# lesliegaga/GPT-SoVITS

Measured on AMD Instinct MI355X. Metric: synthesised audio sec/sec (1/RTF), v2 pipeline, higher is better.
Workload: dtype f16

## Files before the change

gpt-sovits_amd/csrc/conv_wide.hip:

```cpp
#include <stdio.h>
#include <stdlib.h>

#include <algorithm>
#include <type_traits>

#include "common.h"

namespace gsv {

namespace {

typedef _Float16 T;
typedef h8 F;
typedef _Float16 T4 __attribute__((ext_vector_type(4)));

__device__ __forceinline__ void mma32w(f16v& acc, const h8& a, const h8& b) { acc = __builtin_amdgcn_mfma_f32_32x32x16_f16(a, b, acc, 0, 0, 0); }
__device__ __forceinline__ h8 lrelu8w(h8 v, float s) { h8 t = v * (_Float16)s; return __builtin_elementwise_max(v, t); }
__device__ __forceinline__ h8 relu8w(h8 v) { return __builtin_elementwise_max(v, (h8){0, 0, 0, 0, 0, 0, 0, 0}); }

template <bool RES, bool ACCU, int NW>
__global__ __launch_bounds__(NW * 64) void conv_wide_f16_kernel(ConvArgs a, int rows_win, int ntiles) {
  constexpr int G = 8, KC = 16, CC = 128, CT = 128, TM = 2, TN = NW == 8 ? 2 : 4, WN = NW == 8 ? 4 : 2, NT = NW * 64;
  constexpr int LDX = CC + G, VPR = CC / G;
  constexpr int WLOADS = CT * VPR / NT;
  constexpr int XB = (306 * VPR + NT - 1) / NT;
  constexpr int LDO = CT + 4, PR = TN * 32, IPR = CT / 4, NI = PR * IPR / NT;
  extern __shared__ __attribute__((aligned(16))) unsigned char smem[];
  T* xs = (T*)smem;
  T* ws = xs + (size_t)306 * LDX;
  float* os = (float*)smem;
  static_assert((size_t)PR * LDO * 4 <= (size_t)306 * LDX * 2, "epilogue tile must fit in the window");
  const int tid = threadIdx.x, lane = tid & 63, wave = tid >> 6;
  const int r = lane & 31, h = lane >> 5;
  const int wm = wave / WN, wn = wave % WN;
  const T* __restrict__ x = (const T*)a.x;
  const T* __restrict__ w = (const T*)a.w;
  const int total = rows_win * VPR;
  const int ecg = tid % IPR, ec = 4 * ecg;
  f4 ebias = (f4){0.f, 0.f, 0.f, 0.f};
  if (a.bias) for (int j = 0; j < 4; ++j) ebias[j] = a.bias[ec + j];

  auto load_w = [&](int tap, F* regs) {
#pragma unroll
    for (int i = 0; i < WLOADS; ++i) {
      const int v = tid + i * NT;
      const int row = v / VPR, col = v - row * VPR;
      regs[i] = *(const F*)(w + (long long)row * a.ldw + (long long)tap * CC + col * G);
    }
  };
  auto store_w = [&](int buf, const F* regs) {
#pragma unroll
    for (int i = 0; i < WLOADS; ++i) {
      const int v = tid + i * NT;
      const int row = v / VPR, col = v - row * VPR;
      *(F*)(ws + ((size_t)buf * CT + row) * LDX + col * G) = regs[i];
    }
  };
  auto load_window = [&](int tile, F* regs) {
    const int win_start = tile * 256 - a.pad;
#pragma unroll
    for (int i = 0; i < XB; ++i) {
      const int v = min(tid + i * NT, total - 1);
      const int row = v / VPR, col = v - row * VPR;
      const int ti = win_start + row;
      const F val = *(const F*)(x + (long long)min(max(ti, 0), a.T_in - 1) * a.ldx + col * G);
      regs[i] = (ti >= 0 && ti < a.T_in) ? val : (F){0, 0, 0, 0, 0, 0, 0, 0};
    }
  };
  auto store_window = [&](const F* regs) {
#pragma unroll
    for (int i = 0; i < XB; ++i) {
      const int v = tid + i * NT;
      if (v < total) {
        const int row = v / VPR, col = v - row * VPR;
        F val = regs[i];
        if (a.pre_act == ACT_LRELU) val = lrelu8w(val, a.pre_slope);
        else if (a.pre_act == ACT_RELU) val = relu8w(val);
        *(F*)(xs + (size_t)row * LDX + col * G) = val;
      }
    }
  };
  int tile = blockIdx.x;
  {
    F first[XB], w0[WLOADS];
    load_window(min(tile, ntiles - 1), first);
    load_w(0, w0);
    store_window(first);
    store_w(0, w0);
  }
  lds_barrier();
  for (; tile < ntiles; tile += gridDim.x) {
    const int t0 = tile * 256;
    const bool pf = a.prof && blockIdx.x == 100 && tile == 100 + 3 * (int)gridDim.x && tid == 0;
    int pi = 0;
#define WSTAMP() do { if (pf) a.prof[pi++] = __builtin_amdgcn_s_memrealtime(); } while (0)
    WSTAMP();
    F nxt[XB];
    load_window(min(tile + (int)gridDim.x, ntiles - 1), nxt);
    T4 rv[RES ? NI : 1];
    auto load_res_pass = [&](int pass) {
#pragma unroll
      for (int e = 0; e < (RES ? NI : 0); ++e) {
        const int t = min(t0 + pass * PR + (tid + e * NT) / IPR, a.T_out - 1);
        rv[e] = *(const T4*)((const T*)a.res + (long long)t * a.ldr + ec);
      }
    };
    if (RES) load_res_pass(0);
    f16v acc[TM][TN];
#pragma unroll
    for (int m = 0; m < TM; ++m)
#pragma unroll
      for (int n = 0; n < TN; ++n)
#pragma unroll
        for (int i = 0; i < 16; ++i) acc[m][n][i] = 0.f;
    for (int tap = 0; tap < a.taps; ++tap) {
      const int buf = tap & 1;
      F wnx[WLOADS];
      const bool more = tap + 1 < a.taps;
      if (more) load_w(tap + 1, wnx);
      const int shift = tap * a.dil;
      const T* wb = ws + (size_t)buf * CT * LDX;
#pragma unroll 2
      for (int ks = 0; ks < CC / KC; ++ks) {
        const int kk = ks * KC + G * h;
        F af[TM], bf[TN];
#pragma unroll
        for (int m = 0; m < TM; ++m) af[m] = *(const F*)(wb + (size_t)((wm * TM + m) * 32 + r) * LDX + kk);
#pragma unroll
        for (int n = 0; n < TN; ++n) bf[n] = *(const F*)(xs + (size_t)((wn * TN + n) * 32 + r + shift) * LDX + kk);
#pragma unroll
        for (int m = 0; m < TM; ++m)
#pragma unroll
          for (int n = 0; n < TN; ++n) mma32w(acc[m][n], af[m], bf[n]);
      }
      if (more) {
        store_w(buf ^ 1, wnx);
        lds_barrier();
      }
      WSTAMP();
    }
#pragma unroll
    for (int pass = 0; pass < WN; ++pass) {
      lds_barrier();
      WSTAMP();
      if (wn == pass) {
#pragma unroll
        for (int m = 0; m < TM; ++m)
#pragma unroll
          for (int n = 0; n < TN; ++n) {
            const int tl = n * 32 + r;
#pragma unroll
            for (int g = 0; g < 4; ++g) {
              const int cl = (wm * TM + m) * 32 + 8 * g + 4 * h;
              *(f4*)(os + (size_t)tl * LDO + cl) = (f4){acc[m][n][4 * g], acc[m][n][4 * g + 1], acc[m][n][4 * g + 2], acc[m][n][4 * g + 3]};
            }
          }
      }
      WSTAMP();
      lds_barrier();
      WSTAMP();
      T4 ya[ACCU ? NI : 1];
#pragma unroll
      for (int e = 0; e < (ACCU ? NI : 0); ++e) {
        const int t = min(t0 + pass * PR + (tid + e * NT) / IPR, a.T_out - 1);
        ya[e] = *(const T4*)((const T*)a.y + (long long)t * a.ldy + ec);
      }
      auto items = [&](auto act_tag) {
#pragma unroll
        for (int e = 0; e < NI; ++e) {
          const int tl = (tid + e * NT) / IPR;
          const int t = t0 + pass * PR + tl;
          if (t >= a.T_out) continue;
          const f4 av = *(const f4*)(os + (size_t)tl * LDO + 4 * ecg);
          float v[4];
#pragma unroll
          for (int j = 0; j < 4; ++j) {
            float u = av[j] + ebias[j];
            if (RES) u += (float)rv[e][j];
            u *= a.scale;
            u = post_act_c<decltype(act_tag)::value>(a.post_act, u);
            if (ACCU) u += (float)ya[e][j];
            v[j] = u;
          }
          *(T4*)((T*)a.y + (long long)t * a.ldy + ec) = (T4){(T)v[0], (T)v[1], (T)v[2], (T)v[3]};
        }
      };
      GSV_ACT_DISPATCH(a.post_act, items);
      if (RES && pass + 1 < WN) load_res_pass(pass + 1);
      WSTAMP();
    }
    F w0[WLOADS];
    load_w(0, w0);
    lds_barrier();
    store_window(nxt);
    store_w(0, w0);
    lds_barrier();
    WSTAMP();
  }
}

}

int launch_conv_wide(int dtype, const ConvArgs& a, hipStream_t s) {
  static const bool off = getenv("GSV_NO_CONV_WIDE") != nullptr;
  if (off || dtype != GSV_F16) return 1;
  if (a.Cin != 128 || a.Cout != 128 || a.Z != 1 || a.stride != 1 || a.ups_u > 0 || a.dil < 1 || a.gate || a.taps < 2) return 1;
  if (a.out_f32 || a.res_f32 || a.y_col0 != 0 || a.T_virt < 16384 || a.T_out != a.T_virt || a.T_in < 1) return 1;
  if (a.ldx % 8 != 0 || a.ldw % 8 != 0 || a.ldy % 4 != 0 || (a.res && a.ldr % 4 != 0) || ((uintptr_t)a.x % 16) || ((uintptr_t)a.w % 16)) return 1;
  const int span = (a.taps - 1) * a.dil;
  if (span > 50 || a.pad < 0 || a.pad > span) return 1;
  const int rows_win = 256 + span;
  const int ntiles = cdiv(a.T_virt, 256);
  const size_t lds = ((size_t)306 + 2 * 128) * 136 * 2;
  const int grid = std::min(ntiles, 256);
  ConvArgs b = a;
  static unsigned long long* d_prof = nullptr;
  static int prof_calls = 0;
  if (getenv("GSV_WIDE_PROF") && !d_prof) { (void)hipMalloc((void**)&d_prof, 64 * 8); (void)hipMemset(d_prof, 0, 64 * 8); }
  b.prof = d_prof;
  const bool res = a.res != nullptr, acc = a.accumulate != 0;
  static const int nw = getenv("GSV_WIDE_WAVES") ? atoi(getenv("GSV_WIDE_WAVES")) : 8;
#define GSV_WIDE_NW(R, A, W)                                                                                               \
  do {                                                                                                                     \
    auto kern = conv_wide_f16_kernel<R, A, W>;                                                                             \
    static bool set = false;                                                                                               \
    if (!set) { GSV_HIP(hipFuncSetAttribute((const void*)kern, hipFuncAttributeMaxDynamicSharedMemorySize, 160 * 1024)); set = true; } \
    hipLaunchKernelGGL(kern, dim3(grid), dim3(W * 64), lds, s, b, rows_win, ntiles);                                       \
  } while (0)
#define GSV_WIDE(R, A) do { if (nw == 8) GSV_WIDE_NW(R, A, 8); else GSV_WIDE_NW(R, A, 4); } while (0)
  if (res && acc) GSV_WIDE(true, true);
  else if (res) GSV_WIDE(true, false);
  else if (acc) GSV_WIDE(false, true);
  else GSV_WIDE(false, false);
#undef GSV_WIDE
#undef GSV_WIDE_NW
  GSV_HIP(hipGetLastError());
  if (d_prof && ++prof_calls == 3) {
    (void)hipStreamSynchronize(s);
    unsigned long long hp[64];
    (void)hipMemcpy(hp, d_prof, sizeof(hp), hipMemcpyDeviceToHost);
    fprintf(stderr, "[wide prof] taps %d:", a.taps);
    for (int i = 1; i < 24 && hp[i]; ++i) fprintf(stderr, " %.2f", (double)(hp[i] - hp[0]) / 100.0);
    fprintf(stderr, "\n");
  }
  return GSV_OK;
}

}
```

Before: 2789.

## Add persistent ring-pipelined conv kernel for 128/256-channel dilated convolutions

Adds a new persistent conv kernel that double-buffers weight slabs per tap and spreads the next tile's input window loads across the taps. This overlaps global loads with MFMA work. It extends coverage to Cin/Cout of 256 by looping over input-channel chunks and splitting output halves across blocks, and it reuses a weight slab for the epilogue staging. It runs first by default for 3/7/11-tap convs, with the old wide kernel kept as a fallback. The risks are extra barriers per tap and higher register pressure from the per-tap template unrolling.

```diff
diff --git a/gpt-sovits_amd/csrc/conv_wide.hip b/gpt-sovits_amd/csrc/conv_wide.hip
--- a/gpt-sovits_amd/csrc/conv_wide.hip
+++ b/gpt-sovits_amd/csrc/conv_wide.hip
@@ -3,6 +3,7 @@
 
 #include <algorithm>
 #include <type_traits>
+#include <utility>
 
 #include "common.h"
 
@@ -197,13 +198,271 @@
     lds_barrier();
     WSTAMP();
   }
-}
-
+#undef WSTAMP
+}
+
+template <int... I, class Fn> __device__ __forceinline__ void static_for(std::integer_sequence<int, I...>, Fn&& f) {
+  (f(std::integral_constant<int, I>{}), ...);
+}
+
+template <bool RES, bool ACCU, int TAPS>
+__global__ __launch_bounds__(512) void conv_ring_f16_kernel(ConvArgs a, int rows_win, int ntiles, int nch, int nh) {
+  constexpr int NW = 8, G = 8, KC = 16, CC = 128, CT = 128, TM = 2, TN = 2, WN = 4, NT = NW * 64;
+  constexpr int LDX = CC + G, VPR = CC / G;
+  constexpr int WLOADS = CT * VPR / NT;
+  constexpr int XB = (306 * VPR + NT - 1) / NT;
+  constexpr int LDO = CT + 4, PR = TN * 32, IPR = CT / 4, NI = PR * IPR / NT;
+  extern __shared__ __attribute__((aligned(16))) unsigned char smem[];
+  T* xs = (T*)smem;
+  T* ws = xs + (size_t)306 * LDX;
+  static_assert((size_t)PR * LDO * 4 <= (size_t)CT * LDX * 2, "epilogue pass must fit in a weight slab");
+  const int tid = threadIdx.x, lane = tid & 63, wave = tid >> 6;
+  const int r = lane & 31, h = lane >> 5;
+  const int wm = wave / WN, wn = wave % WN;
+  const T* __restrict__ x = (const T*)a.x;
+  const T* __restrict__ w = (const T*)a.w;
+  const int total = rows_win * VPR;
+  const int half = nh == 2 ? (blockIdx.x >> 3) & 1 : 0;
+  const int cout0 = half * CT;
+  const int tstep = nh == 2 ? (int)gridDim.x / 2 : (int)gridDim.x;
+  int tile = nh == 2 ? (blockIdx.x >> 4) * 8 + (blockIdx.x & 7) : blockIdx.x;
+  if (tile >= ntiles) return;
+  const int ecg = tid % IPR, ec = cout0 + 4 * ecg;
+
+  auto opaque = [](int v) { asm volatile("" : "+s"(v)); return v; };
+  auto load_w = [&](int tap, int c, F* regs) {
+    const int ldw = opaque(a.ldw);
+#pragma unroll
+    for (int i = 0; i < WLOADS; ++i) {
+      const int v = tid + i * NT;
+      const int row = v / VPR, col = v - row * VPR;
+      regs[i] = *(const F*)(w + (long long)(cout0 + row) * ldw + (long long)tap * a.Cin + c * CC + col * G);
+    }
+  };
+  auto store_w = [&](int buf, const F* regs) {
+#pragma unroll
+    for (int i = 0; i < WLOADS; ++i) {
+      const int v = tid + i * NT;
+      const int row = v / VPR, col = v - row * VPR;
+      *(F*)(ws + ((size_t)buf * CT + row) * LDX + col * G) = regs[i];
+    }
+  };
+  auto load_window = [&](int tl, int c, F* regs, auto i0, auto i1) {
+    const int win_start = tl * 256 - a.pad;
+    const int ldx = opaque(a.ldx);
+#pragma unroll
+    for (int i = decltype(i0)::value; i < decltype(i1)::value; ++i) {
+      const int v = min(tid + i * NT, total - 1);
+      const int row = v / VPR, col = v - row * VPR;
+      const int ti = win_start + row;
+      regs[i] = *(const F*)(x + (long long)min(max(ti, 0), a.T_in - 1) * ldx + c * CC + col * G);
+    }
+  };
+  auto store_window = [&](int tl, const F* regs) {
+    const int win_start = tl * 256 - a.pad;
+#pragma unroll
+    for (int i = 0; i < XB; ++i) {
+      const int v = tid + i * NT;
+      if (v < total) {
+        const int row = v / VPR, col = v - row * VPR;
+        const int ti = win_start + row;
+        F val = (ti >= 0 && ti < a.T_in) ? regs[i] : (F){0, 0, 0, 0, 0, 0, 0, 0};
+        if (a.pre_act == ACT_LRELU) val = lrelu8w(val, a.pre_slope);
+        else if (a.pre_act == ACT_RELU) val = relu8w(val);
+        *(F*)(xs + (size_t)row * LDX + col * G) = val;
+      }
+    }
+  };
+  {
+    F first[XB], w0[WLOADS];
+    load_window(tile, 0, first, std::integral_constant<int, 0>{}, std::integral_constant<int, XB>{});
+    load_w(0, 0, w0);
+    store_window(tile, first);
+    store_w(0, w0);
+  }
+  lds_barrier();
+  int pbuf = 0;
+  for (int it = 0; tile < ntiles; tile += tstep, ++it) {
+    const int t0 = tile * 256;
+    const bool pf = a.prof && blockIdx.x == 100 && it == 1 && tid == 0;
+    int pi = 0;
+#define RSTAMP() do { if (pf) a.prof[pi++] = __builtin_amdgcn_s_memrealtime(); } while (0)
+    RSTAMP();
+    const int ntile = tile + tstep < ntiles ? tile + tstep : tile;
+    T4 rv[RES ? NI : 1], yv[ACCU ? NI : 1];
+    f4 ebias = (f4){0.f, 0.f, 0.f, 0.f};
+    auto load_epi_pass = [&](int pass) {
+#pragma unroll
+      for (int e = 0; e < NI; ++e) {
+        const int t = min(t0 + pass * PR + (tid + e * NT) / IPR, a.T_out - 1);
+        if (RES) rv[e] = *(const T4*)((const T*)a.res + (long long)t * a.ldr + ec);
+        if (ACCU && !RES) yv[e] = *(const T4*)((const T*)a.y + (long long)t * a.ldy + ec);
+      }
+    };
+    f16v acc[TM][TN];
+#pragma unroll
+    for (int m = 0; m < TM; ++m)
+#pragma unroll
+      for (int n = 0; n < TN; ++n)
+#pragma unroll
+        for (int i = 0; i < 16; ++i) acc[m][n][i] = 0.f;
+    int last_buf = 0;
+    for (int c = 0; c < nch; ++c) {
+      const bool last = c + 1 == nch;
+      const int nc = last ? 0 : c + 1, nt = last ? ntile : tile;
+      F nxt[XB];
+      static_for(std::make_integer_sequence<int, TAPS>{}, [&](auto tap_c) {
+        constexpr int tap = decltype(tap_c)::value;
+        const int buf = pbuf ^ (tap & 1);
+        F wnx[WLOADS];
+        if (tap + 1 < TAPS) load_w(tap + 1, c, wnx);
+        else load_w(0, nc, wnx);
+        load_window(nt, nc, nxt, std::integral_constant<int, tap * XB / TAPS>{}, std::integral_constant<int, (tap + 1) * XB / TAPS>{});
+        if (tap == TAPS - 2 && last) {
+          if (a.bias) ebias = *(const f4*)(a.bias + ec);
+          load_epi_pass(0);
+        }
+        const int shift = tap * opaque(a.dil);
+        const T* wb = ws + (size_t)buf * CT * LDX;
+#pragma unroll 2
+        for (int ks = 0; ks < CC / KC; ++ks) {
+          const int kk = ks * KC + G * h;
+          F af[TM], bf[TN];
+#pragma unroll
+          for (int m = 0; m < TM; ++m) af[m] = *(const F*)(wb + (size_t)((wm * TM + m) * 32 + r) * LDX + kk);
+#pragma unroll
+          for (int n = 0; n < TN; ++n) bf[n] = *(const F*)(xs + (size_t)((wn * TN + n) * 32 + r + shift) * LDX + kk);
+#pragma unroll
+          for (int m = 0; m < TM; ++m)
+#pragma unroll
+            for (int n = 0; n < TN; ++n) mma32w(acc[m][n], af[m], bf[n]);
+        }
+        if (tap + 1 < TAPS) {
+          store_w(buf ^ 1, wnx);
+          lds_barrier();
+        } else {
+          lds_barrier();
+          store_window(nt, nxt);
+          store_w(buf ^ 1, wnx);
+          last_buf = buf;
+          if (!last) lds_barrier();
+        }
+        RSTAMP();
+      });
+      pbuf = last_buf ^ 1;
+    }
+    float* os = (float*)(ws + (size_t)last_buf * CT * LDX);
+#pragma unroll
+    for (int pass = 0; pass < WN; ++pass) {
+      if (pass > 0) lds_barrier();
+      if (wn == pass) {
+#pragma unroll
+        for (int m = 0; m < TM; ++m)
+#pragma unroll
+          for (int n = 0; n < TN; ++n) {
+            const int tl = n * 32 + r;
+#pragma unroll
+            for (int g = 0; g < 4; ++g) {
+              const int cl = (wm * TM + m) * 32 + 8 * g + 4 * h;
+              *(f4*)(os + (size_t)tl * LDO + cl) = (f4){acc[m][n][4 * g], acc[m][n][4 * g + 1], acc[m][n][4 * g + 2], acc[m][n][4 * g + 3]};
+            }
+          }
+      }
+      lds_barrier();
+      if (ACCU && RES) {
+#pragma unroll
+        for (int e = 0; e < NI; ++e) {
+          const int t = min(t0 + pass * PR + (tid + e * NT) / IPR, a.T_out - 1);
+          yv[e] = *(const T4*)((const T*)a.y + (long long)t * a.ldy + ec);
+        }
+      }
+      auto items = [&](auto act_tag) {
+#pragma unroll
+        for (int e = 0; e < NI; ++e) {
+          const int tl = (tid + e * NT) / IPR;
+          const int t = t0 + pass * PR + tl;
+          if (t >= a.T_out) continue;
+          const f4 av = *(const f4*)(os + (size_t)tl * LDO + 4 * ecg);
+          float v[4];
+#pragma unroll
+          for (int j = 0; j < 4; ++j) {
+            float u = av[j] + ebias[j];
+            if (RES) u += (float)rv[e][j];
+            u *= a.scale;
+            u = post_act_c<decltype(act_tag)::value>(a.post_act, u);
+            if (ACCU) u += (float)yv[e][j];
+            v[j] = u;
+          }
+          *(T4*)((T*)a.y + (long long)t * a.ldy + ec) = (T4){(T)v[0], (T)v[1], (T)v[2], (T)v[3]};
+        }
+      };
+      GSV_ACT_DISPATCH(a.post_act, items);
+      if ((RES || ACCU) && pass + 1 < WN) load_epi_pass(pass + 1);
+    }
+    lds_barrier();
+    RSTAMP();
+#undef RSTAMP
+  }
+}
+
+}
+
+static void print_prof(const char* name, const ConvArgs& a, unsigned long long* d_prof, hipStream_t s) {
+  (void)hipStreamSynchronize(s);
+  unsigned long long hp[64];
+  (void)hipMemcpy(hp, d_prof, sizeof(hp), hipMemcpyDeviceToHost);
+  fprintf(stderr, "[%s prof] Cin %d Cout %d taps %d dil %d (us after the tile's start):", name, a.Cin, a.Cout, a.taps, a.dil);
+  for (int i = 1; i < 64 && hp[i]; ++i) fprintf(stderr, " %.2f", (double)(hp[i] - hp[0]) / 100.0);
+  fprintf(stderr, "\n");
+}
+
+static int launch_conv_ring(const ConvArgs& a, hipStream_t s) {
+  if ((a.Cin != 128 && a.Cin != 256) || (a.Cout != 128 && a.Cout != 256) || a.Z != 1 || a.stride != 1 || a.ups_u > 0 || a.gate) return 1;
+  if (a.taps != 3 && a.taps != 7 && a.taps != 11) return 1;
+  if (a.accumulate) return 1;
+  if (a.dil < 1 || a.dil > 5 || a.out_f32 || a.res_f32 || a.y_col0 != 0 || a.T_virt < 16384 || a.T_out != a.T_virt || a.T_in < 1) return 1;
+  if (a.ldx % 8 != 0 || a.ldx < a.Cin || a.ldw % 8 != 0 || a.ldw < a.taps * a.Cin || a.ldy % 4 != 0 || a.ldy < a.Cout ||
+      (a.res && (a.ldr % 4 != 0 || a.ldr < a.Cout)) || ((uintptr_t)a.x % 16) || ((uintptr_t)a.w % 16) || ((uintptr_t)a.y % 8) ||
+      (a.res && ((uintptr_t)a.res % 8)) || ((uintptr_t)a.bias % 16))
+    return 1;
+  const int span = (a.taps - 1) * a.dil;
+  if (a.pad < 0 || a.pad > span) return 1;
+  const int rows_win = 256 + span;
+  const int ntiles = cdiv(a.T_virt, 256);
+  const int nch = a.Cin / 128, nh = a.Cout / 128;
+  const int grid = nh == 2 ? std::min(cdiv(ntiles, 8) * 16, 256) : std::min(ntiles, 256);
+  const size_t lds = ((size_t)306 + 2 * 128) * 136 * 2;
+  ConvArgs b = a;
+  static unsigned long long* d_prof = nullptr;
+  static int prof_calls = 0;
+  if (getenv("GSV_WIDE_PROF") && !d_prof) { (void)hipMalloc((void**)&d_prof, 64 * 8); (void)hipMemset(d_prof, 0, 64 * 8); }
+  b.prof = d_prof;
+  const bool res = a.res != nullptr;
+#define GSV_RING_T(R, A, K)                                                                                                \
+  do {                                                                                                                     \
+    auto kern = conv_ring_f16_kernel<R, A, K>;                                                                             \
+    static bool set = false;                                                                                               \
+    if (!set) { GSV_HIP(hipFuncSetAttribute((const void*)kern, hipFuncAttributeMaxDynamicSharedMemorySize, 160 * 1024)); set = true; } \
+    hipLaunchKernelGGL(kern, dim3(grid), dim3(512), lds, s, b, rows_win, ntiles, nch, nh);                                 \
+  } while (0)
+#define GSV_RING(R, A) do { if (a.taps == 3) GSV_RING_T(R, A, 3); else if (a.taps == 7) GSV_RING_T(R, A, 7); else GSV_RING_T(R, A, 11); } while (0)
+  if (res) GSV_RING(true, false);
+  else GSV_RING(false, false);
+#undef GSV_RING
+#undef GSV_RING_T
+  GSV_HIP(hipGetLastError());
+  if (d_prof && ++prof_calls == 3) print_prof("ring", a, d_prof, s);
+  return GSV_OK;
 }
 
 int launch_conv_wide(int dtype, const ConvArgs& a, hipStream_t s) {
   static const bool off = getenv("GSV_NO_CONV_WIDE") != nullptr;
+  static const bool no_ring = getenv("GSV_NO_CONV_RING") != nullptr;
   if (off || dtype != GSV_F16) return 1;
+  if (!no_ring) {
+    const int rc = launch_conv_ring(a, s);
+    if (rc <= 0) return rc;
+  }
   if (a.Cin != 128 || a.Cout != 128 || a.Z != 1 || a.stride != 1 || a.ups_u > 0 || a.dil < 1 || a.gate || a.taps < 2) return 1;
   if (a.out_f32 || a.res_f32 || a.y_col0 != 0 || a.T_virt < 16384 || a.T_out != a.T_virt || a.T_in < 1) return 1;
   if (a.ldx % 8 != 0 || a.ldw % 8 != 0 || a.ldy % 4 != 0 || (a.res && a.ldr % 4 != 0) || ((uintptr_t)a.x % 16) || ((uintptr_t)a.w % 16)) return 1;
@@ -235,15 +494,9 @@
 #undef GSV_WIDE
 #undef GSV_WIDE_NW
   GSV_HIP(hipGetLastError());
-  if (d_prof && ++prof_calls == 3) {
-    (void)hipStreamSynchronize(s);
-    unsigned long long hp[64];
-    (void)hipMemcpy(hp, d_prof, sizeof(hp), hipMemcpyDeviceToHost);
-    fprintf(stderr, "[wide prof] taps %d:", a.taps);
-    for (int i = 1; i < 24 && hp[i]; ++i) fprintf(stderr, " %.2f", (double)(hp[i] - hp[0]) / 100.0);
-    fprintf(stderr, "\n");
-  }
+  if (d_prof && ++prof_calls == 3) print_prof("wide", a, d_prof, s);
   return GSV_OK;
 }
 
-}
+
+}
```

After: 2817, median of 6. Within noise of the previous version (+1.0%).
